# samivout/clair-torch

Hardware: AMD Instinct MI355X
Metric: MPix/s HDR-merged (+uncertainty) at N=32 4K RGB (higher is better)
Workload: dtype f32; 1 GPU; C2: 32-exposure 4096x4096x3 uint16 stack per GPU, merge+uncertainty (LINEAR ICRF 3x256, Gaussian weights, sigma: multiplier, float64 mean + float32 std out); global_image=4096x4096x3 in 1 row band(s)

## Files before the change

clair_torch_amd/csrc/ct_merge_exact.hip:

```cpp
#include <algorithm>
#include <cstdlib>
#include "ct_merge.hpp"

namespace ct {

struct TorchRowSum {
    float a0 = 0.0f, a1 = 0.0f, a2 = 0.0f, a3 = 0.0f;
    __device__ __forceinline__ void add(float v, int row)
    {
        a0 = a0 + v;
        const int n = row + 1;
        if ((n & 15) == 0) {
            a1 = a1 + a0;
            a0 = 0.0f;
            if ((n & 0xf0) == 0) {
                a2 = a2 + a1;
                a1 = 0.0f;
                if ((n & 0xf00) == 0) {
                    a3 = a3 + a2;
                    a2 = 0.0f;
                }
            }
        }
    }
    __device__ __forceinline__ float total() const { return ((a0 + a1) + a2) + a3; }
};

__device__ __forceinline__ float exp_correctly_rounded(float v)
{
    const double x = (double)v;
    const double k = __builtin_rint(x * 1.4426950408889634);
    double r = __builtin_fma(k, -0x1.62e42fefa38p-1, x);
    r = __builtin_fma(k, -0x1.ef35793c7673p-45, r);
    double p = 2.755731922398589e-07;
    p = __builtin_fma(p, r, 2.7557319223985893e-06);
    p = __builtin_fma(p, r, 2.48015873015873e-05);
    p = __builtin_fma(p, r, 1.984126984126984e-04);
    p = __builtin_fma(p, r, 1.3888888888888889e-03);
    p = __builtin_fma(p, r, 8.333333333333333e-03);
    p = __builtin_fma(p, r, 4.1666666666666664e-02);
    p = __builtin_fma(p, r, 1.6666666666666666e-01);
    p = __builtin_fma(p, r, 0.5);
    p = __builtin_fma(p, r, 1.0);
    p = __builtin_fma(p, r, 1.0);
    const double kk = k < -1100.0 ? -1100.0 : k;
    return (float)__builtin_ldexp(p, (int)kk);
}

__device__ __forceinline__ float sqrt_correctly_rounded(float v)
{
    if (!(v > 0.0f) || v > 3.0e38f) return __builtin_sqrtf(v);
    float s = (float)__builtin_sqrt((double)v);
    const double vd = (double)v;
    const float up = __uint_as_float(__float_as_uint(s) + 1u), dn = __uint_as_float(__float_as_uint(s) - 1u);
    const double m_up = 0.5 * ((double)s + (double)up), m_dn = 0.5 * ((double)s + (double)dn);
    if (m_up * m_up < vd)
        s = up;
    else if (m_dn * m_dn > vd)
        s = dn;
    return s;
}

template <typename T, int V, int INTERP, int WEIGHT, int STD, int CACHE = 0>
__global__ __launch_bounds__(kBlock) void merge_reference_order_kernel(const MergeArgs a, const MergeBatches mb)
{
    extern __shared__ __align__(16) char lds[];
    constexpr bool kGauss = WEIGHT == CT_WEIGHT_GAUSS;
    constexpr bool kHasStd = STD != CT_STD_NONE;
    constexpr int kEntry = lut_entry_bytes(INTERP);
    const int C = a.channels, L = a.n_points;
    const int n_exposures = a.batch;
    stage_lut<INTERP, false>(lds, a.lut, C, L);
    double *inv_t = reinterpret_cast<double *>(lds + ((INTERP == CT_INTERP_NONE ? 0 : C * L * kEntry) + 7 & ~7));
    for (int n = threadIdx.x; n < n_exposures; n += kBlock) inv_t[n] = 1.0 / a.exposure[n];
    int b_max = n_exposures;
    if (mb.n_batches > 0) {
        b_max = 0;
        for (int k = 0; k < mb.n_batches; ++k) b_max = mb.batch_size[k] > b_max ? mb.batch_size[k] : b_max;
    }
    [[maybe_unused]] float *wc = reinterpret_cast<float *>(inv_t + n_exposures) + threadIdx.x;
    [[maybe_unused]] float *lc = wc + (size_t)b_max * V * kBlock;
    __syncthreads();
    const float top = INTERP == CT_INTERP_NONE ? 1.0f : (float)(L - 1);
    const bool fresh = a.flags & CT_MERGE_FIRST_BATCH, finalize = a.flags & CT_MERGE_FINALIZE;
    const bool keep_state = a.mean_state != nullptr;

    const uint32_t vec = blockIdx.x * (uint32_t)kBlock + threadIdx.x;
    if (vec * (uint32_t)V >= a.q_count) return;
    const uint32_t q0 = a.q_begin + vec * (uint32_t)V;

    uint32_t qp[V];
    const char *row[V];
#pragma unroll
    for (int e = 0; e < V; ++e) {
        qp[e] = a.out_index(q0 + e);
        int ch;
        uint32_t qg;
        a.tile.locate(a.tile.planar_index(q0 + e), ch, qg);
        row[e] = lds + (INTERP == CT_INTERP_NONE ? 0 : lut_row<INTERP>(qg, ch, C) * L * kEntry);
    }

    auto forward = [&](T code, const char *r, float &x, float &xm, float &w, float &lin) {
        x = to_pixel<T>(code, a.norm);
        xm = x - 0.5f;
        w = kGauss ? exp_correctly_rounded(-a.weight_scale * (xm * xm)) : 1.0f;
        float unused;
        lin = icrf_sample<INTERP, true, false>(x, r, top, unused);
    };

    double state_mean[V];
    float state_w[V], state_var[V];
#pragma unroll
    for (int e = 0; e < V; ++e) {
        state_mean[e] = fresh ? 0.0 : a.mean_state[qp[e]];
        state_w[e] = fresh ? 0.0f : a.sumw_state[qp[e]];
        state_var[e] = (fresh || !kHasStd) ? 0.0f : a.var_state[qp[e]];
    }
    const int n_batches = mb.n_batches > 0 ? mb.n_batches : 1;
    int n_first = 0;
    for (int bi = 0; bi < n_batches; ++bi) {
    const int B = mb.n_batches > 0 ? mb.batch_size[bi] : n_exposures;
    const T *src = static_cast<const T *>(mb.n_batches > 0 ? mb.batch_ptr[bi] : a.stack) + q0;
    const float *ssrc = STD == CT_STD_EXPLICIT ? (mb.n_batches > 0 ? mb.std_ptr[bi] : a.std_stack) + q0 : nullptr;
    const bool first = fresh && bi == 0;
    const double *inv_tb = inv_t + n_first;

    TorchRowSum Wsum[V];
    double S[V];
#pragma unroll
    for (int e = 0; e < V; ++e) S[e] = 0.0;
    for (int n = 0; n < B; ++n) {
        const Packet<T, V> pk = *reinterpret_cast<const Packet<T, V> *>(src + (int64_t)n * a.image_stride);
        const double it = inv_tb[n];
#pragma unroll
        for (int e = 0; e < V; ++e) {
            float x, xm, w, lin;
            forward(pk.v[e], row[e], x, xm, w, lin);
            if constexpr (CACHE >= 1) wc[(n * V + e) * kBlock] = w;
            if constexpr (CACHE == 2) lc[(n * V + e) * kBlock] = lin;
            const double y = (double)lin * it;
            Wsum[e].add(w, n);
            S[e] = S[e] + (double)w * y;
        }
    }

    float Wb[V], D[V], Wt[V], frac[V], g_wb[V], var_in[V];
    double mean[V], g_s[V];
#pragma unroll
    for (int e = 0; e < V; ++e) {
        Wb[e] = Wsum[e].total();
        D[e] = Wb[e] + 1e-6f;
        const double mb = S[e] / (double)D[e];
        const float WA = first ? 0.0f : state_w[e];
        const double meanA = first ? 0.0 : state_mean[e];
        Wt[e] = WA + Wb[e];
        frac[e] = __fdiv_rn(Wb[e], Wt[e]);
        const double diff = mb - meanA;
        mean[e] = meanA + (double)frac[e] * diff;
        var_in[e] = (first || !kHasStd) ? 0.0f : state_var[e];
        if constexpr (kHasStd) {
            const float g_frac = (float)diff;
            g_s[e] = (double)frac[e] / (double)D[e];
            const float g_d = (float)(-(double)frac[e] * ((S[e] / (double)D[e]) / (double)D[e]));
            float g = __fdiv_rn(g_frac, Wt[e]);
            g = g + (-g_frac * __fdiv_rn(__fdiv_rn(Wb[e], Wt[e]), Wt[e]));
            g_wb[e] = g + g_d;
        }
    }

    float var_o[V];
    if constexpr (kHasStd) {
        TorchRowSum U[V];
        for (int n = 0; n < B; ++n) {
            const Packet<T, V> pk = *reinterpret_cast<const Packet<T, V> *>(src + (int64_t)n * a.image_stride);
            Packet<float, V> sp;
            if constexpr (STD == CT_STD_EXPLICIT) sp = *reinterpret_cast<const Packet<float, V> *>(ssrc + (int64_t)n * a.image_stride);
            const double it = inv_tb[n];
#pragma unroll
            for (int e = 0; e < V; ++e) {
                float x, xm, w, lin;
                if constexpr (CACHE == 0) {
                    forward(pk.v[e], row[e], x, xm, w, lin);
                } else {
                    x = to_pixel<T>(pk.v[e], a.norm);
                    xm = x - 0.5f;
                    w = wc[(n * V + e) * kBlock];
                    if constexpr (CACHE == 2) {
                        lin = lc[(n * V + e) * kBlock];
                    } else {
                        float unused;
                        lin = icrf_sample<INTERP, true, false>(x, row[e], top, unused);
                    }
                }
                const double y = (double)lin * it;
                const float g_lin = (float)((g_s[e] * (double)w) * it);
                float g_x = icrf_grad_reference_order<INTERP>(x, row[e], top, g_lin);
                if constexpr (kGauss) {
                    const float g_w = (float)(g_s[e] * y) + g_wb[e];
                    const float g_a = ((g_w * w) * -a.weight_scale) * (2.0f * xm);
                    g_x = INTERP == CT_INTERP_LOOKUP ? g_a : g_x + g_a;
                }
                float sigma = a.std_value;
                if constexpr (STD == CT_STD_MULTIPLIER) sigma = x * a.std_value;
                if constexpr (STD == CT_STD_EXPLICIT) sigma = sp.v[e];
                const float gs = g_x * sigma;
                U[e].add(gs * gs, n);
            }
        }
#pragma unroll
        for (int e = 0; e < V; ++e) var_o[e] = first ? U[e].total() : var_in[e] + U[e].total();
    }

#pragma unroll
    for (int e = 0; e < V; ++e) {
        state_mean[e] = mean[e];
        state_w[e] = Wt[e];
        if constexpr (kHasStd) state_var[e] = var_o[e];
    }
    n_first += B;
    }

#pragma unroll
    for (int e = 0; e < V; ++e) {
        if (keep_state) {
            a.mean_state[qp[e]] = state_mean[e];
            a.sumw_state[qp[e]] = state_w[e];
            if constexpr (kHasStd) a.var_state[qp[e]] = state_var[e];
        }
        if (finalize) {
            if (a.flags & CT_MERGE_MEAN_OUT_F32)
                static_cast<float *>(a.mean_out)[qp[e]] = (float)state_mean[e];
            else
                static_cast<double *>(a.mean_out)[qp[e]] = state_mean[e];
            if constexpr (kHasStd) a.std_out[qp[e]] = sqrt_correctly_rounded(state_var[e]);
        }
    }
}

static size_t exact_fixed_lds(const MergeArgs &a, int interp)
{
    return (lut_lds_bytes(interp, a.channels, a.n_points) + 7 & ~(size_t)7) +
           sizeof(double) * (size_t)a.batch;
}

constexpr size_t kCacheBudgetBoth = 37 * 1024, kCacheBudgetWeight = 45 * 1024;
static int exact_cache_level(const MergeArgs &a, int b_max, int interp, int weight_mode, int std_mode, int v)
{
    if (std_mode == CT_STD_NONE) return 0;
    static const bool disabled = getenv("CT_EXACT_NO_CACHE") != nullptr;
    if (disabled) return 0;
    const size_t per_level = (size_t)b_max * v * kBlock * sizeof(float);
    if (exact_fixed_lds(a, interp) + 2 * per_level <= kCacheBudgetBoth) return 2;
    if (weight_mode == CT_WEIGHT_GAUSS && exact_fixed_lds(a, interp) + per_level <= kCacheBudgetWeight) return 1;
    return 0;
}

struct ExactRoute {
    MergeBatches mb;
    int b_max;
};

template <typename T, int V, int INTERP, int WEIGHT, int STD, int CACHE = 0>
static int exact_launch(const MergeArgs &a, const ExactRoute &r, hipStream_t s)
{
    if (a.q_count == 0) return CT_OK;
    const uint32_t vecs = (a.q_count + V - 1) / V, grid = (vecs + kBlock - 1) / kBlock;
    const size_t lds = exact_fixed_lds(a, INTERP) + (size_t)CACHE * r.b_max * V * kBlock * sizeof(float);
    if (lds > kLdsBudget) return CT_ERR_TOO_LARGE;
    hipLaunchKernelGGL((merge_reference_order_kernel<T, V, INTERP, WEIGHT, STD, CACHE>), dim3(grid), dim3(kBlock), lds, s, a, r.mb);
    return hipGetLastError() == hipSuccess ? CT_OK : CT_ERR_LAUNCH;
}

template <typename T, int V, int INTERP, int WEIGHT>
static int exact_std(const MergeArgs &a, const ExactRoute &r, int std_mode, hipStream_t s)
{
    if constexpr (V == 4) {
        const int level = exact_cache_level(a, r.b_max, INTERP, WEIGHT, std_mode, V);
        if (level == 2) {
            switch (std_mode) {
                case CT_STD_CONSTANT: return exact_launch<T, V, INTERP, WEIGHT, CT_STD_CONSTANT, 2>(a, r, s);
                case CT_STD_MULTIPLIER: return exact_launch<T, V, INTERP, WEIGHT, CT_STD_MULTIPLIER, 2>(a, r, s);
                case CT_STD_EXPLICIT: return exact_launch<T, V, INTERP, WEIGHT, CT_STD_EXPLICIT, 2>(a, r, s);
            }
        } else if (level == 1) {
            switch (std_mode) {
                case CT_STD_CONSTANT: return exact_launch<T, V, INTERP, WEIGHT, CT_STD_CONSTANT, 1>(a, r, s);
                case CT_STD_MULTIPLIER: return exact_launch<T, V, INTERP, WEIGHT, CT_STD_MULTIPLIER, 1>(a, r, s);
                case CT_STD_EXPLICIT: return exact_launch<T, V, INTERP, WEIGHT, CT_STD_EXPLICIT, 1>(a, r, s);
            }
        }
    }
    switch (std_mode) {
        case CT_STD_NONE: return exact_launch<T, V, INTERP, WEIGHT, CT_STD_NONE>(a, r, s);
        case CT_STD_CONSTANT: return exact_launch<T, V, INTERP, WEIGHT, CT_STD_CONSTANT>(a, r, s);
        case CT_STD_MULTIPLIER: return exact_launch<T, V, INTERP, WEIGHT, CT_STD_MULTIPLIER>(a, r, s);
        case CT_STD_EXPLICIT: return exact_launch<T, V, INTERP, WEIGHT, CT_STD_EXPLICIT>(a, r, s);
    }
    return CT_ERR_INVALID_ARGUMENT;
}

template <typename T, int V>
static int exact_interp(const MergeArgs &a, const ExactRoute &r, int interp, int weight_mode, int std_mode, hipStream_t s)
{
    const bool gauss = weight_mode == CT_WEIGHT_GAUSS;
    switch (interp) {
        case CT_INTERP_LOOKUP:
            return gauss ? exact_std<T, V, CT_INTERP_LOOKUP, CT_WEIGHT_GAUSS>(a, r, std_mode, s)
                         : exact_std<T, V, CT_INTERP_LOOKUP, CT_WEIGHT_NONE>(a, r, std_mode, s);
        case CT_INTERP_LINEAR:
            return gauss ? exact_std<T, V, CT_INTERP_LINEAR, CT_WEIGHT_GAUSS>(a, r, std_mode, s)
                         : exact_std<T, V, CT_INTERP_LINEAR, CT_WEIGHT_NONE>(a, r, std_mode, s);
        case CT_INTERP_CATMULL:
            return gauss ? exact_std<T, V, CT_INTERP_CATMULL, CT_WEIGHT_GAUSS>(a, r, std_mode, s)
                         : exact_std<T, V, CT_INTERP_CATMULL, CT_WEIGHT_NONE>(a, r, std_mode, s);
        case CT_INTERP_NONE:
            return gauss ? exact_std<T, V, CT_INTERP_NONE, CT_WEIGHT_GAUSS>(a, r, std_mode, s)
                         : exact_std<T, V, CT_INTERP_NONE, CT_WEIGHT_NONE>(a, r, std_mode, s);
    }
    return CT_ERR_INVALID_ARGUMENT;
}

template <typename T>
static int exact_typed(MergeArgs a, const ExactRoute &r, uint32_t Q, int interp, int weight_mode, int std_mode, hipStream_t s)
{
    constexpr int V = 4;
    bool vec_ok = aligned(a.stack, sizeof(T) * V) && (a.image_stride % V) == 0 && aligned(a.std_stack, 4 * V);
    for (int b = 0; b < r.mb.n_batches; ++b) vec_ok = vec_ok && aligned(r.mb.batch_ptr[b], sizeof(T) * V) && aligned(r.mb.std_ptr[b], 4 * V);
    const uint32_t q_vec = vec_ok ? (Q / V) * V : 0;
    int rc = CT_OK;
    if (q_vec) {
        a.q_begin = 0;
        a.q_count = q_vec;
        rc = exact_interp<T, V>(a, r, interp, weight_mode, std_mode, s);
        if (rc != CT_OK) return rc;
    }
    if (q_vec < Q) {
        a.q_begin = q_vec;
        a.q_count = Q - q_vec;
        rc = exact_interp<T, 1>(a, r, interp, weight_mode, std_mode, s);
    }
    return rc;
}

int merge_reference_order(const MergeArgs &a, int dtype, uint32_t q_total, int interp, int weight_mode, int std_mode,
                          hipStream_t stream, const MergeBatches *batches)
{
    if (a.batch > 65536) return CT_ERR_TOO_LARGE;
    ExactRoute r{};
    r.b_max = a.batch;
    if (batches && batches->n_batches > 0) {
        if (batches->n_batches > kMaxMergeBatches) return CT_ERR_INVALID_ARGUMENT;
        r.mb = *batches;
        r.b_max = 0;
        for (int b = 0; b < batches->n_batches; ++b) r.b_max = std::max(r.b_max, (int)batches->batch_size[b]);
    }
    switch (dtype) {
        case CT_DTYPE_U8: return exact_typed<uint8_t>(a, r, q_total, interp, weight_mode, std_mode, stream);
        case CT_DTYPE_U16: return exact_typed<uint16_t>(a, r, q_total, interp, weight_mode, std_mode, stream);
        case CT_DTYPE_F32: return exact_typed<float>(a, r, q_total, interp, weight_mode, std_mode, stream);
    }
    return CT_ERR_UNSUPPORTED;
}

}
```

Before: 20190 MPix/s.

## Cache per-exposure weights in registers with software prefetch for small stacks

Adds a register-cache variant for Gaussian-weighted merges with at most 32 exposures and 4-wide packets, used when the LDS caches do not fit. The first pass stores the weights in a fully unrolled register array, and the uncertainty pass reuses them instead of recomputing the Gaussian. Both passes prefetch the next exposure packet one iteration ahead. The kernel is limited to 2 waves per EU to make room for the registers, which lowers occupancy and latency hiding.

Measured after the change: 20140 MPix/s. Within noise of the previous version (-0.2%).

```diff
diff --git a/clair_torch_amd/csrc/ct_merge_exact.hip b/clair_torch_amd/csrc/ct_merge_exact.hip
--- a/clair_torch_amd/csrc/ct_merge_exact.hip
+++ b/clair_torch_amd/csrc/ct_merge_exact.hip
@@ -61,8 +61,11 @@
     return s;
 }
 
+constexpr int kRegChunk = 32;
+
 template <typename T, int V, int INTERP, int WEIGHT, int STD, int CACHE = 0>
-__global__ __launch_bounds__(kBlock) void merge_reference_order_kernel(const MergeArgs a, const MergeBatches mb)
+__global__ __launch_bounds__(kBlock) __attribute__((amdgpu_waves_per_eu(CACHE == 3 ? 2 : 1, CACHE == 3 ? 2 : 8)))
+void merge_reference_order_kernel(const MergeArgs a, const MergeBatches mb)
 {
     extern __shared__ __align__(16) char lds[];
     constexpr bool kGauss = WEIGHT == CT_WEIGHT_GAUSS;
@@ -129,6 +132,26 @@
     double S[V];
 #pragma unroll
     for (int e = 0; e < V; ++e) S[e] = 0.0;
+    [[maybe_unused]] float wr[CACHE == 3 ? kRegChunk : 1][V];
+    if constexpr (CACHE == 3) {
+        Packet<T, V> ahead = *reinterpret_cast<const Packet<T, V> *>(src);
+#pragma unroll
+        for (int n = 0; n < kRegChunk; ++n) {
+            if (n < B) {
+                const Packet<T, V> pk = ahead;
+                ahead = *reinterpret_cast<const Packet<T, V> *>(src + (int64_t)(n + 1 < B ? n + 1 : B - 1) * a.image_stride);
+                const double it = inv_tb[n];
+#pragma unroll
+                for (int e = 0; e < V; ++e) {
+                    float x, xm, lin;
+                    forward(pk.v[e], row[e], x, xm, wr[n][e], lin);
+                    const double y = (double)lin * it;
+                    Wsum[e].add(wr[n][e], n);
+                    S[e] = S[e] + (double)wr[n][e] * y;
+                }
+            }
+        }
+    } else
     for (int n = 0; n < B; ++n) {
         const Packet<T, V> pk = *reinterpret_cast<const Packet<T, V> *>(src + (int64_t)n * a.image_stride);
         const double it = inv_tb[n];
@@ -171,6 +194,44 @@
     float var_o[V];
     if constexpr (kHasStd) {
         TorchRowSum U[V];
+        if constexpr (CACHE == 3) {
+            auto cached_sample = [&](int n, int e, T code, float w, float sigma_explicit, double it) {
+                const float x = to_pixel<T>(code, a.norm), xm = x - 0.5f;
+                float unused;
+                const float lin = icrf_sample<INTERP, true, false>(x, row[e], top, unused);
+                const double y = (double)lin * it;
+                const float g_lin = (float)((g_s[e] * (double)w) * it);
+                float g_x = icrf_grad_reference_order<INTERP>(x, row[e], top, g_lin);
+                const float g_w = (float)(g_s[e] * y) + g_wb[e];
+                const float g_a = ((g_w * w) * -a.weight_scale) * (2.0f * xm);
+                g_x = INTERP == CT_INTERP_LOOKUP ? g_a : g_x + g_a;
+                float sigma = a.std_value;
+                if constexpr (STD == CT_STD_MULTIPLIER) sigma = x * a.std_value;
+                if constexpr (STD == CT_STD_EXPLICIT) sigma = sigma_explicit;
+                const float gs = g_x * sigma;
+                U[e].add(gs * gs, n);
+            };
+            auto load_std = [&](int n) {
+                Packet<float, V> sp{};
+                if constexpr (STD == CT_STD_EXPLICIT) sp = *reinterpret_cast<const Packet<float, V> *>(ssrc + (int64_t)n * a.image_stride);
+                return sp;
+            };
+            Packet<T, V> ahead = *reinterpret_cast<const Packet<T, V> *>(src);
+            Packet<float, V> sahead = load_std(0);
+#pragma unroll
+            for (int n = 0; n < kRegChunk; ++n) {
+                if (n < B) {
+                    const Packet<T, V> pk = ahead;
+                    const Packet<float, V> sp = sahead;
+                    const int next = n + 1 < B ? n + 1 : B - 1;
+                    ahead = *reinterpret_cast<const Packet<T, V> *>(src + (int64_t)next * a.image_stride);
+                    sahead = load_std(next);
+                    const double it = inv_tb[n];
+#pragma unroll
+                    for (int e = 0; e < V; ++e) cached_sample(n, e, pk.v[e], wr[n][e], sp.v[e], it);
+                }
+            }
+        } else
         for (int n = 0; n < B; ++n) {
             const Packet<T, V> pk = *reinterpret_cast<const Packet<T, V> *>(src + (int64_t)n * a.image_stride);
             Packet<float, V> sp;
@@ -252,6 +313,7 @@
     const size_t per_level = (size_t)b_max * v * kBlock * sizeof(float);
     if (exact_fixed_lds(a, interp) + 2 * per_level <= kCacheBudgetBoth) return 2;
     if (weight_mode == CT_WEIGHT_GAUSS && exact_fixed_lds(a, interp) + per_level <= kCacheBudgetWeight) return 1;
+    if (weight_mode == CT_WEIGHT_GAUSS && v == 4 && b_max <= kRegChunk) return 3;
     return 0;
 }
 
@@ -265,7 +327,7 @@
 {
     if (a.q_count == 0) return CT_OK;
     const uint32_t vecs = (a.q_count + V - 1) / V, grid = (vecs + kBlock - 1) / kBlock;
-    const size_t lds = exact_fixed_lds(a, INTERP) + (size_t)CACHE * r.b_max * V * kBlock * sizeof(float);
+    const size_t lds = exact_fixed_lds(a, INTERP) + (size_t)(CACHE == 3 ? 0 : CACHE) * r.b_max * V * kBlock * sizeof(float);
     if (lds > kLdsBudget) return CT_ERR_TOO_LARGE;
     hipLaunchKernelGGL((merge_reference_order_kernel<T, V, INTERP, WEIGHT, STD, CACHE>), dim3(grid), dim3(kBlock), lds, s, a, r.mb);
     return hipGetLastError() == hipSuccess ? CT_OK : CT_ERR_LAUNCH;
@@ -287,6 +349,14 @@
                 case CT_STD_CONSTANT: return exact_launch<T, V, INTERP, WEIGHT, CT_STD_CONSTANT, 1>(a, r, s);
                 case CT_STD_MULTIPLIER: return exact_launch<T, V, INTERP, WEIGHT, CT_STD_MULTIPLIER, 1>(a, r, s);
                 case CT_STD_EXPLICIT: return exact_launch<T, V, INTERP, WEIGHT, CT_STD_EXPLICIT, 1>(a, r, s);
+            }
+        } else if (level == 3) {
+            if constexpr (WEIGHT == CT_WEIGHT_GAUSS) {
+                switch (std_mode) {
+                    case CT_STD_CONSTANT: return exact_launch<T, V, INTERP, WEIGHT, CT_STD_CONSTANT, 3>(a, r, s);
+                    case CT_STD_MULTIPLIER: return exact_launch<T, V, INTERP, WEIGHT, CT_STD_MULTIPLIER, 3>(a, r, s);
+                    case CT_STD_EXPLICIT: return exact_launch<T, V, INTERP, WEIGHT, CT_STD_EXPLICIT, 3>(a, r, s);
+                }
             }
         }
     }
```
